# Nicolo2277/Vivim

Measured on AMD Instinct MI355X. Metric: frames/sec fwd+bwd, 256x256 clip=5 3-class, higher is better.
Workload: dtype bf16

## Files before the change

### vivim_amd/_lib.py

```python
import collections
import ctypes
import os
import re
import subprocess

import torch

_HERE = os.path.dirname(os.path.abspath(__file__))
CSRC = os.path.join(_HERE, "csrc")
SO_PATH = os.environ.get("VIVIM_LIB") or os.path.join(CSRC, "libvivim_hip.so")
HEADER = os.path.join(os.path.dirname(_HERE), "include", "vivim_hip.h")

i32, i64, vp = ctypes.c_int32, ctypes.c_int64, ctypes.c_void_p

STRUCT_NAMES = {
    "vivim_ssm_fwd_params": "SsmFwdParams", "vivim_ssm_bwd_params": "SsmBwdParams",
    "vivim_conv_fwd_params": "ConvFwdParams", "vivim_conv_bwd_params": "ConvBwdParams",
    "vivim_dwconv_params": "DwConvParams", "vivim_dwconv_wgrad_params": "DwConvWgradParams",
    "vivim_dir_params": "DirParams", "vivim_conv_update_params": "ConvUpdateParams",
    "vivim_state_update_params": "StateUpdateParams", "vivim_layernorm_params": "LayerNormParams",
    "vivim_wgrad_nt_params": "WgradNtParams", "vivim_add_layernorm_params": "AddLayerNormParams",
    "vivim_seg_loss_params": "SegLossParams", "vivim_seg_metrics_params": "SegMetricsParams",
    "vivim_upsample_params": "UpsampleParams",
    "vivim_decode_head_params": "DecodeHeadParams", "vivim_token_layernorm_params": "TokenLayerNormParams",
    "vivim_token_add_norm_params": "TokenAddNormParams", "vivim_opt_step_params": "OptStepParams",
    "vivim_opt_mw_params": "OptMwParams",
}
EXTENSIONS = {"vivim_hip_ext.h": ({"vivim_structure_loss_params": "StructureLossParams"}, {}),
              "vivim_hip_ext_head.h": ({"vivim_head_concat_params": "HeadConcatParams"}, {}),
              "vivim_hip_ext_binary_metrics.h": ({"vivim_binary_metrics_params": "BinaryMetricsParams"}, {})}

Entry = collections.namedtuple("Entry", "struct extra stream restype")

_FIELD_TYPES = {"int32_t": i32, "int64_t": i64, "float": ctypes.c_float, "double": ctypes.c_double,
                "void *": vp, "const void *": vp, "const void *const *": ctypes.POINTER(vp),
                "const int64_t *": ctypes.POINTER(i64)}
_ARG_TYPES = {"void *": vp, "size_t": ctypes.c_size_t, "int": ctypes.c_int}
_RESTYPES = {"int": ctypes.c_int, "size_t": ctypes.c_size_t, "const char *": ctypes.c_char_p}
_DIRECTIVES = r"\s*#\s*(include|define|ifndef\s+VIVIM_HIP(_[A-Z0-9]+)*_H|endif)\b"


def _refuse(header, what, text):
    raise ValueError(f"{header}: {what}: {' '.join(text.split())!r}")


def _ctype(text):
    return re.sub(r"\s*\*\s*", " *", " ".join(text.split()))


def _declarator(text, table, context, header):
    m = re.fullmatch(r"([\w\s*]*?)(\w+)\s*(?:\[\s*(\d+)\s*\])?", text.strip())
    if not m:
        _refuse(header, "cannot parse the declarator", context)
    if _ctype(m[1]) not in table:
        _refuse(header, f"unknown type {_ctype(m[1])!r}", context)
    ctype = table[_ctype(m[1])]
    return m[2], (ctype * int(m[3]) if m[3] else ctype)


def _has_sizeof_row(cls):
    return cls._fields_[0][0] != "struct_bytes"


def parse_header(text, names=STRUCT_NAMES, header="vivim_hip.h"):
    text = re.sub(r"/\*.*?\*/", " ", text, flags=re.S)
    consts = {k: int(v) for k, v in re.findall(r"^[ \t]*#[ \t]*define[ \t]+(VIVIM_\w+)[ \t]+(-?\d+)[ \t]*$", text, flags=re.M)}
    by_c_name = {}

    def struct(m):
        body, c_name = m[1], m[2]
        if "{" in body or "#" in body:
            _refuse(header, "nested braces or a preprocessor line in a struct", m[0])
        if c_name not in names:
            _refuse(header, "a struct without a Python name in STRUCT_NAMES", c_name)
        types = {**_FIELD_TYPES, **by_c_name}
        fields = []
        for stmt in filter(None, (s.strip() for s in body.split(";"))):
            base = re.match(r"(?:const\s+)?\w+", stmt) or _refuse(header, "cannot parse the field", stmt)
            first, *more = stmt.split(",")
            for decl in [first] + [f"{base[0]} {d}" for d in more]:
                fields.append(_declarator(decl, types, stmt, header))
        by_c_name[c_name] = type(names[c_name], (ctypes.Structure,), {"_fields_": fields, "__module__": __name__})
        return " "

    def enum(m):
        for item in filter(None, (s.strip() for s in m[1].split(","))):
            kv = re.fullmatch(r"(\w+)\s*=\s*(-?\d+)", item) or _refuse(header, "cannot parse the enumerator", item)
            consts[kv[1]] = int(kv[2])
        return " "

    text = re.sub(r"typedef\s+struct\s*\{(.*?)\}\s*(\w+)\s*;", struct, text, flags=re.S)
    text = re.sub(r"(?:typedef\s+)?enum\s*\{([^{}]*)\}\s*\w*\s*;", enum, text)
    missing = [c for c in names if c not in by_c_name]
    if missing:
        _refuse(header, "STRUCT_NAMES names structs the header does not have", ", ".join(missing))
    text = re.sub(r"^[ \t]*#[ \t]*ifdef[ \t]+__cplusplus\b.*?^[ \t]*#[ \t]*endif\b", " ", text, flags=re.S | re.M)
    for line in re.findall(r"^[ \t]*#.*$", text, flags=re.M):
        if not re.match(_DIRECTIVES, line):
            _refuse(header, "a preprocessor line it does not know", line)
    text = re.sub(r"^[ \t]*#.*$", " ", text, flags=re.M)

    entries = {}
    for decl in filter(None, (s.strip() for s in text.split(";"))):
        m = re.fullmatch(r"([\w\s*]+?)(\w+)\s*\(([\w\s*,]*)\)", decl) or _refuse(header, "cannot parse the declaration", decl)
        if _ctype(m[1]) not in _RESTYPES:
            _refuse(header, f"unknown return type {_ctype(m[1])!r}", decl)
        args = [] if m[3].strip() == "void" else [a.strip() for a in m[3].split(",")]
        stream = bool(args) and re.fullmatch(r"void\s*\*\s*stream", args[-1]) is not None
        args = args[:-1] if stream else args
        params, extra = None, []
        for k, arg in enumerate(args):
            p = re.fullmatch(r"const\s+(vivim_\w+)\s*\*\s*\w+", arg) if k == 0 else None
            if not p:
                extra.append(_declarator(arg, _ARG_TYPES, decl, header)[1])
            elif p[1] not in by_c_name:
                _refuse(header, f"unknown struct {p[1]}", decl)
            elif _has_sizeof_row(by_c_name[p[1]]):
                params = by_c_name[p[1]]
            else:
                extra.append(ctypes.POINTER(by_c_name[p[1]]))
        entries[m[2]] = Entry(params, tuple(extra), stream, _RESTYPES[_ctype(m[1])])
    return consts, {names[c]: by_c_name[c] for c in names}, entries


def _read_header(path=None):
    path = path or HEADER
    try:
        with open(path) as f:
            return f.read()
    except OSError as e:
        raise ImportError(f"{path} cannot be read ({e}): the binding is derived from it") from e


def load_extensions(extensions, include_dir, taken_entries, taken_classes):
    classes, entries = {}, {}
    for file, (names, own) in extensions.items():
        _, new, parsed = parse_header(_read_header(os.path.join(include_dir, file)), names, file)
        bad = [f"{n} does not open with struct_bytes" for n, c in new.items() if _has_sizeof_row(c)]
        bad += [f"another header already declares {n}" for n in parsed if n in taken_entries or n in entries]
        bad += [f"the name {n} is already taken" for n in new if n in taken_classes or n in classes]
        if bad:
            raise ImportError(f"{file}: {'; '.join(bad)}")
        own.update(parsed)
        entries.update(parsed)
        classes.update(new)
    return classes, entries


_consts, _classes, ENTRY_POINTS = parse_header(_read_header())
globals().update(_classes)
STRUCTS = tuple(c for c in _classes.values() if _has_sizeof_row(c))
EXPORTS = tuple(ENTRY_POINTS)
ABI_VERSION = _consts["VIVIM_ABI_VERSION"]
F32, F16, BF16 = _consts["VIVIM_F32"], _consts["VIVIM_F16"], _consts["VIVIM_BF16"]
OPT_CHUNK, OPT_MAX_TENSORS, OPT_STATE_WORDS = (_consts["VIVIM_OPT_" + n] for n in ("CHUNK", "MAX_TENSORS", "STATE_WORDS"))
_classes, _entries = load_extensions(EXTENSIONS, os.path.dirname(HEADER), ENTRY_POINTS, globals())
globals().update(_classes)
ALL_ENTRY_POINTS = {**ENTRY_POINTS, **_entries}

_lib = None


def build(force=False):
    if force:
        subprocess.check_call(["make", "-C", CSRC, "clean"])
    subprocess.check_call(["make", "-C", CSRC, "-j4"])
    return SO_PATH


def lib():
    global _lib
    if _lib is None:
        if not os.path.exists(SO_PATH):
            raise ImportError(
                f"{SO_PATH} is missing: run `python -c 'import __graft_entry__ as g; g.build()'` "
                "(or `make -C vivim_amd/csrc`). vivim_amd has no fallback path.")
        L = ctypes.CDLL(SO_PATH)
        for name, e in ALL_ENTRY_POINTS.items():
            fn = getattr(L, name)
            fn.argtypes = ([ctypes.POINTER(e.struct)] if e.struct else []) + list(e.extra) + ([vp] if e.stream else [])
            fn.restype = e.restype
        if L.vivim_abi_version() != ABI_VERSION:
            raise ImportError("libvivim_hip.so ABI version mismatch")
        for which, st in enumerate(STRUCTS):
            if L.vivim_sizeof(which) != ctypes.sizeof(st):
                raise ImportError(f"struct layout mismatch for {st.__name__}: "
                                  f"C {L.vivim_sizeof(which)} vs ctypes {ctypes.sizeof(st)}")
        _lib = L
    return _lib


_ISIZE = {F32: 4, F16: 2, BF16: 2}


def algorithmic_bytes(name, P):
    name = name.removesuffix("_det")
    f = P.f if isinstance(P, (SsmBwdParams, ConvBwdParams)) else P
    if name.startswith("vivim_opt"):
        if name.endswith("finalise"):
            return 8 * P.total_blocks + 4 * OPT_STATE_WORDS
        n = sum(P.numel[i] for i in range(P.count) if P.grads[i])
        if name.endswith("_mw"):
            return 2 * n + 8 * P.n_blocks if name.endswith("stats_mw") else 28 * n
        return 4 * n + 8 * P.n_blocks if name.endswith("stats") else 28 * n
    if name.startswith("vivim_add_layernorm"):
        n = P.batch * P.seqlen * P.channels
        if not P.weight:
            return n * ((2 if name.endswith("fwd") else 1) * _ISIZE[P.itype] + _ISIZE[P.btype])
        if name.endswith("fwd"):
            return n * (2 * _ISIZE[P.itype] + _ISIZE[P.btype] + _ISIZE[P.otype]) + 8 * P.batch * P.seqlen + 8 * P.channels
        res = (_ISIZE[P.itype] if P.dres else 0) + (_ISIZE[P.otype] if P.dy else 0) + (_ISIZE[P.btype] if P.dbranch else 0)
        return n * (2 * _ISIZE[P.itype] + res) + 8 * P.batch * P.seqlen + 12 * P.channels
    if name.startswith("vivim_token_add_norm"):
        n, b, r = P.rows * P.channels, _ISIZE[P.btype], _ISIZE[P.rtype]
        stats = 8 * P.rows if P.mean and P.weight else 0
        small = (4 * (P.rows // P.rows_per_sample) if P.scale else 0) + (4 * P.channels if P.weight else 0)
        if name.endswith("fwd"):
            small += 4 * P.channels if P.weight and P.bias else 0
            return n * (b + (r if P.res else 0) + (r if P.res_out else 0) + (b if P.weight else 0)) + stats + small
        norm = bool(P.weight and P.dy)
        small += (4 * P.channels if norm and P.dweight else 0) + (4 * P.channels if norm and P.dbias else 0)
        return (n * ((r + b if norm else 0) + (r if P.dres else 0) + (r if P.dres_in else 0) + (b if P.dbranch else 0))
                + (stats if norm else 0) + small)
    if name.startswith("vivim_token_layernorm"):
        n = P.rows * P.channels
        stats = 8 * P.rows if P.mean else 0
        if name.endswith("fwd"):
            return n * (_ISIZE[P.itype] + _ISIZE[P.otype]) + stats
        return n * (2 * _ISIZE[P.itype] + _ISIZE[P.otype]) + stats + 12 * P.channels
    if name.startswith("vivim_decode_head"):
        px = sum(P.map_h[s] * P.map_w[s] for s in range(P.n_maps))
        return (P.batch * (px * P.hidden + P.classes * P.out_h * P.out_w) * _ISIZE[P.itype]
                + 4 * (P.hidden + P.classes * P.hidden + P.classes))
    if name.startswith("vivim_head_concat"):
        px = P.out_h * P.out_w
        maps = sum(P.map_c[s] * (P.map_h[s] * P.map_w[s] + px) for s in range(P.n_maps)) * _ISIZE[P.itype]
        return P.batch * (maps + sum(P.map_c[s] * px for s in range(P.n_maps) if P.keep[s]))
    if name.startswith("vivim_upsample"):
        return P.batch * P.channels * (P.in_h * P.in_w + P.out_h * P.out_w) * _ISIZE[P.itype]
    if name.startswith("vivim_seg_metrics"):
        n = P.batch * P.pixels
        return n * (P.classes * _ISIZE[P.itype] + (8 if P.ttype == 0 else 1) + (1 if P.pred else 0)) + 12 * P.batch * P.classes
    if name.startswith("vivim_structure_loss"):
        n = P.batch * P.height * P.width
        return (n * ((2 if name.endswith("bwd") else 1) * P.classes * _ISIZE[P.itype] + (8 if P.ttype == 0 else 1))
                + 12 * P.batch * P.classes)
    if name.startswith("vivim_seg_loss"):
        n = P.batch * P.pixels
        return (n * ((2 if name.endswith("bwd") else 1) * P.classes * _ISIZE[P.itype] + (8 if P.ttype == 0 else 1))
                + 8 * P.batch * P.classes)
    if name.startswith("vivim_binary_metrics"):
        n = P.batch * P.height * P.width
        return (3 * n * (_ISIZE[P.ptype] + _ISIZE.get(P.gtype, 1)) + P.batch * (72 + (4096 if P.hist else 0))
                + (160 if P.state else 0))
    if name.startswith("vivim_selective_scan"):
        s = _ISIZE[f.itype]
        act = f.batch * f.dim * f.seqlen * s
        bc = (f.batch * f.n_groups * f.dstate * f.seqlen) if f.is_variable_B else f.dim * f.dstate
        has_z = bool(f.z)
        if name.endswith("fwd_lean"):
            return (4 if has_z else 3) * act + 2 * bc * (s if f.is_variable_B else 4) + 4 * (f.dim * f.dstate + 2 * f.dim)
        if name.endswith("fwd"):
            n_act = 3 + (2 if has_z else 0)
            return n_act * act + 2 * bc * (s if f.is_variable_B else 4) + 4 * (f.dim * f.dstate + 2 * f.dim)
        n_act = 5 + (3 if has_z else 0) + (1 if (has_z and f.out_z) else 0)
        return (n_act * act + 2 * bc * (s if f.is_variable_B else 4) + 2 * bc * 4
                + 4 * (2 * f.dim * f.dstate + 4 * f.dim))
    if name.endswith("_update"):
        return 0
    if name.startswith("vivim_dir"):
        return 4 * P.batch * P.channels * P.seqlen * _ISIZE[P.itype]
    if name.startswith("vivim_dwconv"):
# ... 136 lines not shown
```

### vivim_amd/dirmap.py

```python
import torch

from . import _lib
from ._lib import ITYPE


def _params(flat, stacked, nframes, csplit, scale, src, dst):
    B, C, L = flat.shape
    P = _lib.DirParams()
    P.batch, P.channels, P.seqlen, P.nframes, P.csplit, P.itype, P.scale = B, C, L, nframes, csplit, ITYPE[flat.dtype], scale
    P.flat_batch_stride, P.flat_c_stride = flat.stride(0), flat.stride(1)
    P.stk_batch_stride, P.stk_half_stride, P.stk_dir_stride, P.stk_c_stride = (stacked.stride(0), stacked.stride(1),
                                                                               stacked.stride(2), stacked.stride(3))
    P.src, P.dst = src.data_ptr(), dst.data_ptr()
    return P


def _scatter(flat, nframes, csplit, scale):
    if flat.stride(-1) != 1:
        flat = flat.contiguous()
    B, C, L = flat.shape
    stacked = _lib.empty((C // csplit, 3, csplit, B, L), flat.dtype, flat.device).permute(3, 0, 1, 2, 4)
    _lib.launch("vivim_dir_scatter", _params(flat, stacked, nframes, csplit, scale, flat, stacked), flat.device)
    return stacked


def _gather(stacked, nframes, scale, channel_major=False):
    if stacked.stride(-1) != 1:
        stacked = stacked.contiguous()
    B, H, _, csplit, L = stacked.shape
    if channel_major:
        flat = _lib.empty((H * csplit, B, L), stacked.dtype, stacked.device).permute(1, 0, 2)
    else:
        flat = _lib.empty((B, H * csplit, L), stacked.dtype, stacked.device)
    _lib.launch("vivim_dir_gather", _params(flat, stacked, nframes, csplit, scale, stacked, flat), stacked.device)
    return flat


class _StackFn(torch.autograd.Function):
    @staticmethod
    def forward(ctx, xz, nframes, halves):
        ctx.nframes = nframes
        return _scatter(xz, nframes, xz.shape[1] // halves, 1.0)

    @staticmethod
    def backward(ctx, g):
        return _gather(g, ctx.nframes, 1.0), None, None


class _CombineFn(torch.autograd.Function):
    @staticmethod
    def forward(ctx, o3, nframes):
        ctx.nframes = nframes
        B, _, D, L = o3.shape
        return _gather(o3.view(B, 1, 3, D, L), nframes, 1.0 / 3.0, channel_major=True)

    @staticmethod
    def backward(ctx, g):
        B, D, L = g.shape
        return _scatter(g, ctx.nframes, D, 1.0 / 3.0).view(B, 3, D, L), None


def stack_directions(xz, nframes, halves=2):
    return _StackFn.apply(xz, nframes, halves)


def combine_directions(o3, nframes):
    return _CombineFn.apply(o3, nframes)
```

### vivim_amd/dwconv.py

```python
import os

import torch

from . import _lib
from ._lib import ITYPE, ptr


def supported(x, weight):
    if os.environ.get("VIVIM_NO_DWCONV") or not (x.is_cuda and x.dim() == 3 and x.dtype in ITYPE and x.stride(2) == 1):
        return False
    cv = 16 // x.element_size()
    ks = tuple(weight.shape[2:])
    return (weight.shape[1] == 1 and ks in ((3, 3), (3, 3, 3)) and x.shape[2] % cv == 0
            and x.stride(1) % cv == 0 and x.stride(0) % cv == 0 and x.data_ptr() % 16 == 0)


def _taps(weight):
    C = weight.shape[0]
    return weight.detach().reshape(C, -1).t().contiguous().float()


def _aligned(t):
    cv = 16 // t.element_size()
    if t.stride(2) != 1 or t.data_ptr() % 16 or t.stride(1) % cv or t.stride(0) % cv:
# ... 8 lines not shown
    P = _lib.DwConvParams()
    P.batch, P.depth, P.height, P.width, P.channels = B, D, H, W, C
    P.kd, P.itype, P.flip = wt.shape[0] // 9, ITYPE[x.dtype], int(flip)
    P.x_batch_stride, P.x_token_stride = x.stride(0), x.stride(1)
    P.y_batch_stride, P.y_token_stride = y.stride(0), y.stride(1)
    P.x, P.wt, P.y = x.data_ptr(), wt.data_ptr(), y.data_ptr()
    P.bias = ptr(bias)
    P.act = act
    if aux is not None:
        P.aux, P.aux_batch_stride, P.aux_token_stride = aux.data_ptr(), aux.stride(0), aux.stride(1)
    _lib.launch("vivim_dwconv_fwd", P, x.device)
    return y


def _run_wgrad(x, dy, wt, dims, has_bias):
    B, L, C = x.shape
    D, H, W = dims
    acc = _lib.zeros(wt.shape[0] * C + C, x.device)
    P = _lib.DwConvWgradParams()
    P.batch, P.depth, P.height, P.width, P.channels = B, D, H, W, C
    P.kd, P.itype = wt.shape[0] // 9, ITYPE[x.dtype]
    P.x_batch_stride, P.x_token_stride = x.stride(0), x.stride(1)
    P.dy_batch_stride, P.dy_token_stride = dy.stride(0), dy.stride(1)
    P.x, P.dy, P.dwt = x.data_ptr(), dy.data_ptr(), acc.data_ptr()
    P.dbias = acc.data_ptr() + 4 * wt.shape[0] * C if has_bias else None
    if _lib.deterministic():
        nbytes, ws = _lib.workspace("vivim_dwconv_wgrad_det_workspace_bytes", P, x.device)
        _lib.launch("vivim_dwconv_wgrad_det", P, x.device, ptr(ws), nbytes)
    else:
        _lib.launch("vivim_dwconv_wgrad", P, x.device)
    return acc


class DepthwiseConvTokensFn(torch.autograd.Function):
    @staticmethod
    def forward(ctx, x, weight, bias, D, H, W):
        assert x.shape[1] == D * H * W, "token count must equal D*H*W"
        wt = _taps(weight)
        ctx.save_for_backward(x, wt)
        ctx.dims, ctx.wshape, ctx.wdtype = (D, H, W), weight.shape, weight.dtype
        ctx.has_bias = bias is not None
        ctx.bias_dtype = bias.dtype if bias is not None else None
        return _run_fwd(x, wt, bias.detach().float().contiguous() if bias is not None else None, (D, H, W), False)

    @staticmethod
    def backward(ctx, dy):
        x, wt = ctx.saved_tensors
        D, H, W = ctx.dims
        dy = _aligned(dy)
        dx = _run_fwd(dy, wt, None, (D, H, W), True) if ctx.needs_input_grad[0] else None
        C = x.shape[2]
        acc = _run_wgrad(x, dy, wt, (D, H, W), ctx.has_bias)
        dweight = acc[:wt.shape[0] * C].view(wt.shape[0], C).t().reshape(ctx.wshape).to(ctx.wdtype)
        dbias = acc[wt.shape[0] * C:].to(ctx.bias_dtype) if ctx.has_bias else None
        return dx, dweight, dbias, None, None, None


class DepthwiseConvGeluTokensFn(torch.autograd.Function):

    @staticmethod
    def forward(ctx, x, weight, bias, D, H, W):
        assert x.shape[1] == D * H * W, "token count must equal D*H*W"
        wt = _taps(weight)
        bf = bias.detach().float().contiguous() if bias is not None else None
        ctx.save_for_backward(x, wt, bf)
        ctx.dims, ctx.wshape, ctx.wdtype = (D, H, W), weight.shape, weight.dtype
        ctx.bias_dtype = bias.dtype if bias is not None else None
        return _run_fwd(x, wt, bf, (D, H, W), False, act=1)

    @staticmethod
    def backward(ctx, dy):
        x, wt, bf = ctx.saved_tensors
        dims = ctx.dims
        dpre = _run_fwd(x, wt, bf, dims, False, act=2, aux=_aligned(dy))
        dx = _run_fwd(dpre, wt, None, dims, True) if ctx.needs_input_grad[0] else None
        C = x.shape[2]
        acc = _run_wgrad(x, dpre, wt, dims, bf is not None)
        dweight = acc[:wt.shape[0] * C].view(wt.shape[0], C).t().reshape(ctx.wshape).to(ctx.wdtype)
        dbias = acc[wt.shape[0] * C:].to(ctx.bias_dtype) if bf is not None else None
        return dx, dweight, dbias, None, None, None


def depthwise_conv_tokens(x, weight, bias, D, H, W):
    return DepthwiseConvTokensFn.apply(x, weight, bias, D, H, W)


def depthwise_conv_gelu_tokens(x, weight, bias, D, H, W):
    return DepthwiseConvGeluTokensFn.apply(x, weight, bias, D, H, W)
```

### vivim_amd/layernorm.py

```python
import ctypes

import torch

from . import _lib
from ._lib import ITYPE, ptr


def supported(x, weight):
    if _lib.deterministic():
        return False
    if not (x.is_cuda and x.dim() == 3 and x.dtype in ITYPE and weight is not None and weight.dtype == torch.float32):
        return False
    B, L, C = x.shape
    e = 16 // x.element_size()
    return (x.stride(1) == 1 and C <= 512 and L % e == 0 and x.stride(0) % e == 0 and x.stride(2) % e == 0
            and x.data_ptr() % 16 == 0 and x.stride(2) >= L)


def worthwhile(x):
    return x.shape[0] * x.shape[1] >= 4096


def _params(x, out_dtype, eps):
    B, L, C = x.shape
    P = _lib.LayerNormParams()
    P.batch, P.seqlen, P.channels, P.itype, P.otype, P.eps = B, L, C, ITYPE[x.dtype], ITYPE[out_dtype], eps
    P.x_batch_stride, P.x_c_stride = x.stride(0), x.stride(2)
    P.x = x.data_ptr()
    return P


def _norm_forward(P, x, weight, bias, out_dtype):
    B, L, C = x.shape
    y = _lib.empty((B, L, C), out_dtype, x.device)
    stats = _lib.empty((2, B, L), torch.float32, x.device)
    P.y_batch_stride, P.y_token_stride = L * C, C
    P.weight, P.bias = weight.data_ptr(), ptr(bias)
    P.y, P.mean = y.data_ptr(), stats.data_ptr()
    P.rstd = P.mean + 4 * B * L
    return y, stats


def _norm_backward(P, query, dy, weight, stats, out_dtype, has_bias):
    B, L, C = P.batch, P.seqlen, P.channels
    P.weight, P.mean = weight.data_ptr(), stats.data_ptr()
    P.rstd = P.mean + 4 * B * L
    if dy is None:
        return None, None
    if dy.dtype != out_dtype:
        dy = dy.to(out_dtype)
    if dy.stride(2) != 1 or dy.stride(1) < C:
        dy = dy.contiguous()
    P.dy, P.y_batch_stride, P.y_token_stride = dy.data_ptr(), dy.stride(0), dy.stride(1)
    dwb = _lib.zeros(2 * C, stats.device)
    P.dweight = dwb.data_ptr()
    P.dbias = P.dweight + 4 * C if has_bias else None
    ws = _lib.workspace(query, P, stats.device)[1]
    P.workspace = ptr(ws)
    return dwb, (dy, ws)


class _LayerNormCM(torch.autograd.Function):
    @staticmethod
    def forward(ctx, x, weight, bias, eps, out_dtype):
        P = _params(x, out_dtype, eps)
        y, stats = _norm_forward(P, x, weight, bias, out_dtype)
        _lib.launch("vivim_layernorm_cm_fwd", P, x.device)
        ctx.save_for_backward(x, weight, stats)
        ctx.eps, ctx.has_bias, ctx.out_dtype = eps, bias is not None, out_dtype
        return y

    @staticmethod
    def backward(ctx, dy):
        x, weight, stats = ctx.saved_tensors
        B, L, C = x.shape
        dx = _lib.empty((B, C, L), x.dtype, x.device).transpose(1, 2)
        P = _params(x, ctx.out_dtype, ctx.eps)
        P.dx, P.dx_batch_stride, P.dx_c_stride = dx.data_ptr(), C * L, L
        dwb, _alive = _norm_backward(P, "vivim_layernorm_bwd_workspace_bytes", dy, weight, stats, ctx.out_dtype, ctx.has_bias)
        _lib.launch("vivim_layernorm_cm_bwd", P, x.device)
        return dx, dwb[:C], (dwb[C:] if ctx.has_bias else None), None, None


def layer_norm_cm(x, weight, bias, eps=1e-5, out_dtype=None):
    if out_dtype is None:
        out_dtype = torch.float32 if torch.is_autocast_enabled() else x.dtype
    return _LayerNormCM.apply(x, weight, bias, eps, out_dtype)


def _cm_ok(t, e):
    return (t.stride(1) == 1 and t.shape[1] % e == 0 and t.stride(0) % e == 0 and t.stride(2) % e == 0
            and t.data_ptr() % 16 == 0 and t.stride(2) >= t.shape[1])


def add_norm_supported(x, branch, weight=None):
    if _lib.deterministic():
        return False
    if not (x.is_cuda and x.dim() == 3 and x.dtype in ITYPE and branch.device == x.device and branch.shape == x.shape):
        return False
    if weight is not None and weight.dtype != torch.float32:
        return False
    if not (branch.dtype == x.dtype or (x.dtype == torch.float32 and branch.dtype in (torch.float16, torch.bfloat16))):
        return False
    C = x.shape[2]
    return C <= 512 and _cm_ok(x, 16 // x.element_size()) and branch.stride(2) == 1 and branch.stride(1) >= C


def _add_params(x, branch, scale):
    B, L, C = x.shape
    P = _lib.AddLayerNormParams()
    P.batch, P.seqlen, P.channels, P.itype, P.btype, P.otype = B, L, C, ITYPE[x.dtype], ITYPE[branch.dtype], ITYPE[x.dtype]
    P.scale = ptr(scale)
    return P


def _check_scale(scale, x):
    if scale is not None and not (scale.dtype == torch.float32 and scale.shape == (x.shape[0],) and scale.is_contiguous()
                                  and scale.device == x.device):
        raise ValueError("scale must be a contiguous (batch,) float32 tensor on x's device")


def _as_cm(g, like):
    if g.dtype != like.dtype:
        g = g.to(like.dtype)
    if not _cm_ok(g, 16 // g.element_size()):
        g = g.transpose(1, 2).contiguous().transpose(1, 2)
    return g


def _add_forward(x, branch, scale, P):
    B, L, C = x.shape
    x_new = _lib.empty((B, C, L), x.dtype, x.device).transpose(1, 2)
    P.x_batch_stride, P.x_c_stride = x.stride(0), x.stride(2)
    P.x_new_batch_stride, P.x_new_c_stride = C * L, L
    P.branch_batch_stride, P.branch_token_stride = branch.stride(0), branch.stride(1)
    P.x, P.branch, P.x_new = x.data_ptr(), branch.data_ptr(), x_new.data_ptr()
    return x_new


class _AddLayerNormCM(torch.autograd.Function):
    @staticmethod
    def forward(ctx, x, branch, weight, bias, scale, eps, out_dtype):
        P = _add_params(x, branch, scale)
        P.otype, P.eps = ITYPE[out_dtype], eps
        x_new = _add_forward(x, branch, scale, P)
        y, stats = _norm_forward(P, x, weight, bias, out_dtype)
        _lib.launch("vivim_add_layernorm_cm_fwd", P, x.device)
        ctx.save_for_backward(x_new, weight, stats, scale)
        ctx.eps, ctx.has_bias, ctx.out_dtype, ctx.branch_dtype = eps, bias is not None, out_dtype, branch.dtype
        ctx.set_materialize_grads(False)
        return x_new, y

    @staticmethod
    def backward(ctx, dres, dy):
        if dres is None and dy is None:
            return (None,) * 7
        x_new, weight, stats, scale = ctx.saved_tensors
        B, L, C = x_new.shape
        P = _lib.AddLayerNormParams()
        P.batch, P.seqlen, P.channels, P.eps = B, L, C, ctx.eps
        P.itype, P.btype, P.otype = ITYPE[x_new.dtype], ITYPE[ctx.branch_dtype], ITYPE[ctx.out_dtype]
        P.scale = ptr(scale)
        P.x_new_batch_stride, P.x_new_c_stride = x_new.stride(0), x_new.stride(2)
        P.x_new = x_new.data_ptr()
        dwb, _alive = _norm_backward(P, "vivim_add_layernorm_bwd_workspace_bytes", dy, weight, stats, ctx.out_dtype, ctx.has_bias)
        if dres is not None:
            dres = _as_cm(dres, x_new)
            P.dres, P.dres_batch_stride, P.dres_c_stride = dres.data_ptr(), dres.stride(0), dres.stride(2)
        dx = _lib.empty((B, C, L), x_new.dtype, x_new.device).transpose(1, 2)
# ... 358 lines not shown
```

### vivim_amd/mamba_simple.py

```python
import math

import torch
import torch.nn as nn
import torch.nn.functional as F

import os

from .dirmap import combine_directions, stack_directions
from .causal_conv1d_interface import causal_conv1d_fn, causal_conv1d_update
from .selective_scan_interface import mamba_inner_fn_no_out_proj, mamba_inner_grouped_fn_no_out_proj, selective_scan_fn
from .selective_state_update import selective_state_update

_DIRECTIONS = ("", "_b", "_s")
_FUSED = ("conv1d{}.weight", "conv1d{}.bias", "x_proj{}.weight", "dt_proj{}.weight", "dt_proj{}.bias", "A{}_log", "D{}")


class _FusedViews(torch.autograd.Function):

    @staticmethod
    def forward(ctx, nb, *args):
        ctx.nb = nb
        return tuple(b.view_as(b) for b in args[:nb])

    @staticmethod
    def backward(ctx, *gs):
        out = [None] * (1 + ctx.nb)
        for g in gs:
            out += [None, None, None] if g is None else [g[0], g[1], g[2]]
        return tuple(out)


class Mamba(nn.Module):
    def __init__(self, d_model, d_state=16, d_conv=4, expand=2, dt_rank="auto", dt_min=0.001, dt_max=0.1,
                 dt_init="random", dt_scale=1.0, dt_init_floor=1e-4, conv_bias=True, bias=False,
                 use_fast_path=True, layer_idx=None, device=None, dtype=None, bimamba_type="none",
                 nframes=5):
        kw = {"device": device, "dtype": dtype}
        super().__init__()
        assert bimamba_type == "v3", "this fork only builds the tri-directional v3 block (mamba_simple.py:125)"
        self.d_model, self.d_state, self.d_conv, self.expand = d_model, d_state, d_conv, expand
        self.d_inner = int(expand * d_model)
        self.dt_rank = math.ceil(d_model / 16) if dt_rank == "auto" else dt_rank
        self.use_fast_path = use_fast_path
        self.layer_idx = layer_idx
        self.bimamba_type = bimamba_type
        self.nframes = nframes
        self.activation = "silu"

        self.in_proj = nn.Linear(d_model, 2 * self.d_inner, bias=bias, **kw)
        for sfx in _DIRECTIONS:
            self.add_module("conv1d" + sfx, nn.Conv1d(self.d_inner, self.d_inner, kernel_size=d_conv,
                                                      groups=self.d_inner, padding=d_conv - 1,
                                                      bias=conv_bias, **kw))
            self.add_module("x_proj" + sfx, nn.Linear(self.d_inner, self.dt_rank + 2 * d_state, bias=False, **kw))
            dt_proj = nn.Linear(self.dt_rank, self.d_inner, bias=True, **kw)
            self.add_module("dt_proj" + sfx, dt_proj)
            if sfx == "":
                std = self.dt_rank ** -0.5 * dt_scale
                if dt_init == "constant":
                    nn.init.constant_(dt_proj.weight, std)
                elif dt_init == "random":
                    nn.init.uniform_(dt_proj.weight, -std, std)
                else:
                    raise NotImplementedError
                dt = torch.exp(torch.rand(self.d_inner, **kw) * (math.log(dt_max) - math.log(dt_min))
                               + math.log(dt_min)).clamp(min=dt_init_floor)
                with torch.no_grad():
                    dt_proj.bias.copy_(dt + torch.log(-torch.expm1(-dt)))
                dt_proj.bias._no_reinit = True
            A_log = torch.log(torch.arange(1, d_state + 1, dtype=torch.float32, device=device)
                              ).repeat(self.d_inner, 1).contiguous()
            a_name = f"A{sfx}_log"
            self.register_parameter(a_name, nn.Parameter(A_log))
            getattr(self, a_name)._no_weight_decay = True
            d_name = "D" + sfx
            self.register_parameter(d_name, nn.Parameter(torch.ones(self.d_inner, device=device)))
            getattr(self, d_name)._no_weight_decay = True
        self.out_proj = nn.Linear(self.d_inner, d_model, bias=bias, **kw)

    def _fuse(self):
        def param(path):
            obj = self
            for name in path.split("."):
                obj = getattr(obj, name)
            return obj
        bufs, groups = [], []
        for kind in _FUSED:
            ps = [param(kind.format(sfx)) for sfx in _DIRECTIONS]
            if any(p is None for p in ps):
                bufs.append(None)
                groups.append(None)
                continue
            buf = torch.stack([p.data for p in ps])
            for g, p in enumerate(ps):
                p.data = buf[g]
            bufs.append(buf)
            groups.append(ps)
        self._fused = bufs
        self._fused_live = [b for b in bufs if b is not None]
        self._fused_args = self._fused_live + [p for ps in groups if ps is not None for p in ps]
        self._fused_where = []
        for kind, buf in zip(_FUSED, bufs):
            if buf is None:
                continue
            for g, sfx in enumerate(_DIRECTIONS):
                *mods, attr = kind.format(sfx).split(".")
                owner = self
                for name in mods:
                    owner = getattr(owner, name)
                self._fused_where.append((owner._parameters, attr, buf[g].data_ptr(), buf.dtype, buf.device))

    def _fused_params(self):
        where = getattr(self, "_fused_where", None)
        ok = where is not None
        if ok:
            args = self._fused_args
            k = len(self._fused_live)
            for i, (params, attr, ptr, dtype, device) in enumerate(where):
                prm = params.get(attr)
                if prm is not args[k + i] or prm.data_ptr() != ptr or prm.dtype != dtype or prm.device != device:
                    ok = False
                    break
        if not ok:
            self._fuse()
        bufs = self._fused
        views = iter(_FusedViews.apply(len(self._fused_live), *self._fused_args))
        return [None if b is None else next(views) for b in bufs]

    def _inner(self, xz, sfx):
        conv, x_proj, dt_proj = (getattr(self, n + sfx) for n in ("conv1d", "x_proj", "dt_proj"))
        A = -torch.exp(getattr(self, f"A{sfx}_log").float())
        return mamba_inner_fn_no_out_proj(
            xz, conv.weight, conv.bias, x_proj.weight, dt_proj.weight, A, None, None,
            getattr(self, "D" + sfx).float(), delta_bias=dt_proj.bias.float(), delta_softplus=True)

    def forward(self, hidden_states, inference_params=None, nframes=None):
        batch, seqlen, _ = hidden_states.shape
        if inference_params is not None:
            conv_state, ssm_state = self._get_states_from_cache(inference_params, batch)
            if inference_params.seqlen_offset > 0:
                return self.step(hidden_states, conv_state, ssm_state)[0]
            return self._prefill(hidden_states, conv_state, ssm_state)
        nf = self.nframes if nframes is None else nframes
        if seqlen % nf != 0:
            raise ValueError(f"seqlen {seqlen} is not a multiple of nframes {nf}")
        xz = (self.in_proj.weight @ hidden_states.reshape(batch * seqlen, -1).t()
              ).view(2 * self.d_inner, batch, seqlen).transpose(0, 1)
        if self.in_proj.bias is not None:
            xz = xz + self.in_proj.bias.to(xz.dtype)[:, None]
        hw = seqlen // nf
        if os.environ.get("VIVIM_SEPARATE_DIRECTIONS", "0") == "1" or seqlen % 8 != 0:
            return self._forward_separate(xz, batch, seqlen, nf, hw)
        D = self.d_inner
        xz3 = stack_directions(xz, nf)
        conv_w, conv_b, x_proj_w, dt_proj_w, dt_bias, A_log, Dp = self._fused_params()
        A = -torch.exp(A_log.float()).view(3 * D, self.d_state)
        o3 = mamba_inner_grouped_fn_no_out_proj(
            xz3, conv_w.view(3 * D, self.d_conv), conv_b.view(3 * D) if conv_b is not None else None, x_proj_w, dt_proj_w,
            A, Dp.float().view(3 * D), dt_bias.float().view(3 * D), True).view(batch, 3, D, seqlen)
        y = combine_directions(o3, nf).transpose(1, 2)
        return F.linear(y, self.out_proj.weight, self.out_proj.bias)

    def _prefill(self, hidden_states, conv_state, ssm_state):
        batch, seqlen, _ = hidden_states.shape
        xz = (self.in_proj.weight @ hidden_states.reshape(batch * seqlen, -1).t()
              ).view(2 * self.d_inner, batch, seqlen).transpose(0, 1)
        if self.in_proj.bias is not None:
            xz = xz + self.in_proj.bias.to(xz.dtype)[:, None]
        x, z = xz.chunk(2, dim=1)
        with torch.no_grad():
            k = min(seqlen, self.d_conv)
            conv_state.zero_()
            conv_state[:, :, self.d_conv - k:].copy_(x[:, :, seqlen - k:])
        x = causal_conv1d_fn(x, self.conv1d.weight.squeeze(1), self.conv1d.bias, self.activation)
        x_dbl = self.x_proj(x.transpose(1, 2).reshape(batch * seqlen, self.d_inner))
        dt, B, C = torch.split(x_dbl, [self.dt_rank, self.d_state, self.d_state], dim=-1)
        dt = (self.dt_proj.weight @ dt.t()).view(self.d_inner, batch, seqlen).transpose(0, 1)
        B = B.reshape(batch, seqlen, self.d_state).transpose(1, 2).contiguous()
        C = C.reshape(batch, seqlen, self.d_state).transpose(1, 2).contiguous()
        y, last_state = selective_scan_fn(x, dt, -torch.exp(self.A_log.float()), B, C, self.D.float(), z=z,
                                          delta_bias=self.dt_proj.bias.float(), delta_softplus=True, return_last_state=True)
        with torch.no_grad():
            ssm_state.copy_(last_state)
        return self.out_proj(y.transpose(1, 2))

    def _get_states_from_cache(self, inference_params, batch_size, initialize_states=False):
        assert self.layer_idx is not None
        if self.layer_idx not in inference_params.key_value_memory_dict:
            inference_params.key_value_memory_dict[self.layer_idx] = self.allocate_inference_cache(batch_size, 0)
        conv_state, ssm_state = inference_params.key_value_memory_dict[self.layer_idx]
        if initialize_states:
            conv_state.zero_()
            ssm_state.zero_()
        return conv_state, ssm_state

    def _forward_separate(self, xz, batch, seqlen, nf, hw):
        out = self._inner(xz, "")
        out_b = self._inner(xz.flip([-1]), "_b").flip([-1])
        xz_s = xz.reshape(batch, 2 * self.d_inner, nf, hw).transpose(2, 3).reshape(batch, 2 * self.d_inner, seqlen)
        out_s = self._inner(xz_s, "_s")
        out_s = out_s.reshape(batch, self.d_inner, hw, nf).transpose(2, 3).reshape(batch, self.d_inner, seqlen)
        y = (out + out_b + out_s).transpose(1, 2) / 3
        return F.linear(y, self.out_proj.weight, self.out_proj.bias)

    def step(self, hidden_states, conv_state, ssm_state):
        assert hidden_states.shape[1] == 1, "Only support decoding with 1 token at a time for now"
        xz = self.in_proj(hidden_states.squeeze(1))
        x, z = xz.chunk(2, dim=-1)
        x = causal_conv1d_update(x.contiguous(), conv_state, self.conv1d.weight.squeeze(1), self.conv1d.bias, self.activation)
# ... 15 lines not shown
```

Before: 235.9.

## Move autograd nodes for dwconv, direction maps, LayerNorm and fused views into C++

```diff
diff --git a/vivim_amd/_lib.py b/vivim_amd/_lib.py
--- a/vivim_amd/_lib.py
+++ b/vivim_amd/_lib.py
@@ -3,6 +3,7 @@
 import os
 import re
 import subprocess
+import sys
 
 import torch
 
@@ -158,13 +159,16 @@
 globals().update(_classes)
 ALL_ENTRY_POINTS = {**ENTRY_POINTS, **_entries}
 
+NODES_PATH = os.path.join(CSRC, "_vivim_nodes.so")
+
 _lib = None
+_nodes = None
 
 
 def build(force=False):
     if force:
         subprocess.check_call(["make", "-C", CSRC, "clean"])
-    subprocess.check_call(["make", "-C", CSRC, "-j4"])
+    subprocess.check_call(["make", "-C", CSRC, "-j4", "PYTHON=" + sys.executable])
     return SO_PATH
 
 
@@ -188,6 +192,39 @@
                                   f"C {L.vivim_sizeof(which)} vs ctypes {ctypes.sizeof(st)}")
         _lib = L
     return _lib
+
+
+def nodes():
+    global _nodes
+    if _nodes is None:
+        lib()
+        if not os.path.exists(NODES_PATH):
+            raise ImportError(
+                f"{NODES_PATH} is missing: run `python -c 'import __graft_entry__ as g; g.build()'` "
+                "(or `make -C vivim_amd/csrc`). vivim_amd has no fallback path.")
+        import importlib.util
+        spec = importlib.util.spec_from_file_location("_vivim_nodes", NODES_PATH)
+        mod = importlib.util.module_from_spec(spec)
+        spec.loader.exec_module(mod)
+        if mod.abi_version != ABI_VERSION or mod.torch_version != torch.__version__.split("+")[0]:
+            raise ImportError(f"{NODES_PATH} was built for ABI version {mod.abi_version} and torch {mod.torch_version}, not "
+                              f"{ABI_VERSION} and {torch.__version__}: rebuild it (`make -C vivim_amd/csrc`)")
+        _nodes = mod
+    return _nodes
+
+
+_cpp_nodes = os.environ.get("VIVIM_NO_CPP_NODES", "0") in ("0", "") and not os.environ.get("VIVIM_LIB")
+
+
+def cpp_nodes(on):
+    global _cpp_nodes
+    prev, _cpp_nodes = _cpp_nodes, bool(on)
+    return prev
+
+
+def use_cpp_nodes(x):
+    return (_cpp_nodes and not GUARD and (_profile is None or not _profile[1]) and x.is_cuda
+            and x.device.index == torch.cuda.current_device())
 
 
 _ISIZE = {F32: 4, F16: 2, BF16: 2}
diff --git a/vivim_amd/csrc/nodes_flags.py b/vivim_amd/csrc/nodes_flags.py
--- /dev/null
+++ b/vivim_amd/csrc/nodes_flags.py
@@ -0,0 +1,14 @@
+import sys
+import sysconfig
+
+import torch
+from torch.utils import cpp_extension
+
+if sys.argv[1:] == ["compile"]:
+    paths = [sysconfig.get_paths()["include"]] + cpp_extension.include_paths()
+    print(" ".join(f"-isystem {p}" for p in paths), f"-D_GLIBCXX_USE_CXX11_ABI={int(torch._C._GLIBCXX_USE_CXX11_ABI)}")
+elif sys.argv[1:] == ["link"]:
+    libs = ("torch", "torch_cpu", "torch_python", "c10", "c10_hip", "torch_hip")
+    print(" ".join(f"-L{p} -Wl,-rpath,{p}" for p in cpp_extension.library_paths()), " ".join("-l" + n for n in libs))
+else:
+    sys.exit("usage: nodes_flags.py compile|link")
diff --git a/vivim_amd/csrc/torch_nodes.cpp b/vivim_amd/csrc/torch_nodes.cpp
--- /dev/null
+++ b/vivim_amd/csrc/torch_nodes.cpp
@@ -0,0 +1,424 @@
+#include <torch/extension.h>
+
+#include <c10/hip/HIPStream.h>
+#include <torch/csrc/DynamicTypes.h>
+#include <torch/csrc/autograd/python_cpp_function.h>
+#include <torch/csrc/autograd/python_variable.h>
+
+#include <cstring>
+#include <stdexcept>
+#include <string>
+#include <vector>
+
+#include "vivim_hip.h"
+#include "vivim_hip_ext.h"
+#include "vivim_hip_ext_binary_metrics.h"
+#include "vivim_hip_ext_head.h"
+
+namespace {
+
+using at::Tensor;
+using torch::autograd::AutogradContext;
+using torch::autograd::variable_list;
+using OptTensor = c10::optional<Tensor>;
+
+int itype_of(at::ScalarType t) {
+    switch (t) {
+    case at::kFloat: return VIVIM_F32;
+    case at::kHalf: return VIVIM_F16;
+    case at::kBFloat16: return VIVIM_BF16;
+    default: {
+        py::gil_scoped_acquire gil;
+        PyErr_SetObject(PyExc_KeyError, reinterpret_cast<PyObject *>(torch::getTHPDtype(t)));
+        throw py::error_already_set();
+    }
+    }
+}
+
+at::ScalarType dtype_of(int64_t itype) {
+    switch (itype) {
+    case VIVIM_F32: return at::kFloat;
+    case VIVIM_F16: return at::kHalf;
+    case VIVIM_BF16: return at::kBFloat16;
+    default: throw std::invalid_argument("itype must be VIVIM_F32, VIVIM_F16 or VIVIM_BF16");
+    }
+}
+
+const void *ptr(const Tensor &t) { return t.defined() ? t.data_ptr() : nullptr; }
+
+const Tensor &value_or_undefined(const OptTensor &t) {
+    static const Tensor undefined;
+    return t.has_value() ? *t : undefined;
+}
+
+void check_rc(int rc) {
+    if (rc != 0)
+        throw std::runtime_error(vivim_last_error());
+}
+
+void *stream_of(const Tensor &t) { return c10::hip::getCurrentHIPStream(t.get_device()).stream(); }
+
+template <class P> void zero(P &p) { std::memset(&p, 0, sizeof(P)); }
+
+void fill_dwconv(vivim_dwconv_params &P, const Tensor &x, const Tensor &wt, const Tensor &bias, const Tensor &y, int64_t D,
+                 int64_t H, int64_t W, bool flip, int act, const Tensor &aux) {
+    zero(P);
+    P.batch = (int32_t)x.size(0), P.depth = (int32_t)D, P.height = (int32_t)H, P.width = (int32_t)W, P.channels = (int32_t)x.size(2);
+    P.kd = (int32_t)(wt.size(0) / 9), P.itype = itype_of(x.scalar_type()), P.flip = flip;
+    P.x_batch_stride = x.stride(0), P.x_token_stride = x.stride(1);
+    P.y_batch_stride = y.stride(0), P.y_token_stride = y.stride(1);
+    P.x = x.data_ptr(), P.wt = wt.data_ptr(), P.y = y.data_ptr();
+    P.bias = ptr(bias);
+    P.act = act;
+    if (aux.defined())
+        P.aux = aux.data_ptr(), P.aux_batch_stride = aux.stride(0), P.aux_token_stride = aux.stride(1);
+}
+
+void fill_dwconv_wgrad(vivim_dwconv_wgrad_params &P, const Tensor &x, const Tensor &dy, const Tensor &acc, int64_t taps, int64_t D,
+                       int64_t H, int64_t W, bool has_bias) {
+    zero(P);
+    const int64_t C = x.size(2);
+    P.batch = (int32_t)x.size(0), P.depth = (int32_t)D, P.height = (int32_t)H, P.width = (int32_t)W, P.channels = (int32_t)C;
+    P.kd = (int32_t)(taps / 9), P.itype = itype_of(x.scalar_type());
+    P.x_batch_stride = x.stride(0), P.x_token_stride = x.stride(1);
+    P.dy_batch_stride = dy.stride(0), P.dy_token_stride = dy.stride(1);
+    P.x = x.data_ptr(), P.dy = dy.data_ptr(), P.dwt = acc.data_ptr();
+    P.dbias = has_bias ? static_cast<char *>(acc.data_ptr()) + 4 * taps * C : nullptr;
+}
+
+Tensor taps_of(const Tensor &weight) {
+    return weight.detach().reshape({weight.size(0), -1}).t().contiguous().to(at::kFloat);
+}
+
+Tensor aligned(const Tensor &t) {
+    const int64_t cv = 16 / t.element_size();
+    if (t.stride(2) != 1 || reinterpret_cast<uintptr_t>(t.data_ptr()) % 16 || t.stride(1) % cv || t.stride(0) % cv)
+        return t.contiguous();
+    return t;
+}
+
+Tensor dwconv_run_fwd(const Tensor &x, const Tensor &wt, const Tensor &bias, int64_t D, int64_t H, int64_t W, bool flip, int act,
+                      const Tensor &aux) {
+    Tensor y = at::empty({x.size(0), x.size(1), x.size(2)}, x.options());
+    vivim_dwconv_params P;
+    fill_dwconv(P, x, wt, bias, y, D, H, W, flip, act, aux);
+    check_rc(vivim_dwconv_fwd(&P, stream_of(x)));
+    return y;
+}
+
+Tensor dwconv_run_wgrad(const Tensor &x, const Tensor &dy, const Tensor &wt, int64_t D, int64_t H, int64_t W, bool has_bias) {
+    const int64_t C = x.size(2), taps = wt.size(0);
+    Tensor acc = at::zeros({taps * C + C}, x.options().dtype(at::kFloat));
+    vivim_dwconv_wgrad_params P;
+    fill_dwconv_wgrad(P, x, dy, acc, taps, D, H, W, has_bias);
+    if (at::globalContext().deterministicAlgorithms()) {
+        const size_t nbytes = vivim_dwconv_wgrad_det_workspace_bytes(&P);
+        Tensor ws;
+        if (nbytes)
+            ws = at::empty({(int64_t)nbytes}, x.options().dtype(at::kByte));
+        check_rc(vivim_dwconv_wgrad_det(&P, ws.defined() ? ws.data_ptr() : nullptr, nbytes, stream_of(x)));
+    } else {
+        check_rc(vivim_dwconv_wgrad(&P, stream_of(x)));
+    }
+    return acc;
+}
+
+struct DwConvFn : torch::autograd::Function<DwConvFn> {
+    static Tensor forward(AutogradContext *ctx, const Tensor &x, const Tensor &weight, const OptTensor &bias, int64_t D, int64_t H,
+                          int64_t W, bool gelu) {
+        if (x.size(1) != D * H * W) {
+            PyErr_SetString(PyExc_AssertionError, "token count must equal D*H*W");
+            throw py::error_already_set();
+        }
+        Tensor wt = taps_of(weight), bf;
+        if (bias.has_value())
+            bf = bias->detach().to(at::kFloat).contiguous();
+        if (gelu)
+            ctx->save_for_backward({x, wt, bf});
+        else
+            ctx->save_for_backward({x, wt});
+        ctx->saved_data["dims"] = std::vector<int64_t>{D, H, W, gelu, bias.has_value(), (int64_t)weight.scalar_type(),
+                                                       (int64_t)(bias.has_value() ? bias->scalar_type() : at::kFloat)};
+        ctx->saved_data["wshape"] = weight.sizes().vec();
+        return dwconv_run_fwd(x, wt, bf, D, H, W, false, gelu ? 1 : 0, Tensor());
+    }
+
+    static variable_list backward(AutogradContext *ctx, variable_list grads) {
+        const variable_list saved = ctx->get_saved_variables();
+        const Tensor &x = saved[0], &wt = saved[1];
+        const std::vector<int64_t> dims = ctx->saved_data["dims"].toIntVector();
+        const int64_t D = dims[0], H = dims[1], W = dims[2];
+        const bool gelu = dims[3], has_bias = dims[4];
+        Tensor dy = aligned(grads[0]);
+        if (gelu)
+            dy = dwconv_run_fwd(x, wt, saved[2], D, H, W, false, 2, dy);
+        Tensor dx;
+        if (ctx->needs_input_grad(0))
+            dx = dwconv_run_fwd(dy, wt, Tensor(), D, H, W, true, 0, Tensor());
+        const int64_t C = x.size(2), taps = wt.size(0);
+        Tensor acc = dwconv_run_wgrad(x, dy, wt, D, H, W, has_bias);
+        Tensor dweight = acc.slice(0, 0, taps * C).view({taps, C}).t().reshape(ctx->saved_data["wshape"].toIntVector())
+                             .to((at::ScalarType)dims[5]);
+        Tensor dbias;
+        if (has_bias)
+            dbias = acc.slice(0, taps * C).to((at::ScalarType)dims[6]);
+        return {dx, dweight, dbias, Tensor(), Tensor(), Tensor(), Tensor()};
+    }
+};
+
+void fill_dir(vivim_dir_params &P, const Tensor &flat, const Tensor &stacked, int64_t nframes, int64_t csplit, double scale,
+              bool scatter) {
+    zero(P);
+    P.batch = (int32_t)flat.size(0), P.channels = (int32_t)flat.size(1), P.seqlen = (int32_t)flat.size(2);
+    P.nframes = (int32_t)nframes, P.csplit = (int32_t)csplit, P.itype = itype_of(flat.scalar_type()), P.scale = (float)scale;
+    P.flat_batch_stride = flat.stride(0), P.flat_c_stride = flat.stride(1);
+    P.stk_batch_stride = stacked.stride(0), P.stk_half_stride = stacked.stride(1);
+    P.stk_dir_stride = stacked.stride(2), P.stk_c_stride = stacked.stride(3);
+    P.src = scatter ? flat.data_ptr() : stacked.data_ptr();
+    P.dst = scatter ? stacked.data_ptr() : flat.data_ptr();
+}
+
+Tensor dir_scatter(Tensor flat, int64_t nframes, int64_t csplit, double scale) {
+    if (flat.stride(-1) != 1)
+        flat = flat.contiguous();
+    const int64_t B = flat.size(0), C = flat.size(1), L = flat.size(2);
+    Tensor stacked = at::empty({C / csplit, 3, csplit, B, L}, flat.options()).permute({3, 0, 1, 2, 4});
+    vivim_dir_params P;
+    fill_dir(P, flat, stacked, nframes, csplit, scale, true);
+    check_rc(vivim_dir_scatter(&P, stream_of(flat)));
+    return stacked;
+}
+
+Tensor dir_gather(Tensor stacked, int64_t nframes, double scale, bool channel_major) {
+    if (stacked.stride(-1) != 1)
+        stacked = stacked.contiguous();
+    const int64_t B = stacked.size(0), Hh = stacked.size(1), csplit = stacked.size(3), L = stacked.size(4);
+    Tensor flat = channel_major ? at::empty({Hh * csplit, B, L}, stacked.options()).permute({1, 0, 2})
+                                : at::empty({B, Hh * csplit, L}, stacked.options());
+    vivim_dir_params P;
+    fill_dir(P, flat, stacked, nframes, csplit, scale, false);
+    check_rc(vivim_dir_gather(&P, stream_of(stacked)));
+    return flat;
+}
+
+struct StackFn : torch::autograd::Function<StackFn> {
+    static Tensor forward(AutogradContext *ctx, const Tensor &xz, int64_t nframes, int64_t halves) {
+        ctx->saved_data["nframes"] = nframes;
+        return dir_scatter(xz, nframes, xz.size(1) / halves, 1.0);
+    }
+    static variable_list backward(AutogradContext *ctx, variable_list grads) {
+        return {dir_gather(grads[0], ctx->saved_data["nframes"].toInt(), 1.0, false), Tensor(), Tensor()};
+    }
+};
+
+struct CombineFn : torch::autograd::Function<CombineFn> {
+    static Tensor forward(AutogradContext *ctx, const Tensor &o3, int64_t nframes) {
+        ctx->saved_data["nframes"] = nframes;
+        const int64_t B = o3.size(0), D = o3.size(2), L = o3.size(3);
+        return dir_gather(o3.view({B, 1, 3, D, L}), nframes, 1.0 / 3.0, true);
+    }
+    static variable_list backward(AutogradContext *ctx, variable_list grads) {
+        const Tensor &g = grads[0];
+        const int64_t B = g.size(0), D = g.size(1), L = g.size(2);
+        return {dir_scatter(g, ctx->saved_data["nframes"].toInt(), D, 1.0 / 3.0).view({B, 3, D, L}), Tensor()};
+    }
+};
+
+struct FusedViewsFn : torch::autograd::Function<FusedViewsFn> {
+    static variable_list forward(AutogradContext *ctx, int64_t nb, at::TensorList args) {
+        ctx->saved_data["nb"] = nb;
+        variable_list out;
+        out.reserve(nb);
+        for (int64_t i = 0; i < nb; ++i)
+            out.push_back(args[i].view_as(args[i]));
+        return out;
+    }
+    static variable_list backward(AutogradContext *ctx, variable_list grads) {
+        const int64_t nb = ctx->saved_data["nb"].toInt();
+        variable_list out(1 + nb);
+        out.reserve(1 + 4 * nb);
+        for (const Tensor &g : grads)
+            for (int64_t k = 0; k < 3; ++k)
+                out.push_back(g.defined() ? g.select(0, k) : Tensor());
+        return out;
+    }
+};
+
+void fill_layernorm(vivim_layernorm_params &P, const Tensor &x, at::ScalarType out_dtype, double eps) {
+    zero(P);
+    P.batch = (int32_t)x.size(0), P.seqlen = (int32_t)x.size(1), P.channels = (int32_t)x.size(2);
+    P.itype = itype_of(x.scalar_type()), P.otype = itype_of(out_dtype), P.eps = (float)eps;
+    P.x_batch_stride = x.stride(0), P.x_c_stride = x.stride(2);
+    P.x = x.data_ptr();
+}
+
+void fill_layernorm_fwd(vivim_layernorm_params &P, const Tensor &x, const Tensor &weight, const Tensor &bias, const Tensor &y,
+                        const Tensor &stats, at::ScalarType out_dtype, double eps) {
+    fill_layernorm(P, x, out_dtype, eps);
+    const int64_t B = x.size(0), L = x.size(1), C = x.size(2);
+    P.y_batch_stride = L * C, P.y_token_stride = C;
+    P.weight = weight.data_ptr(), P.bias = ptr(bias);
+    P.y = y.data_ptr(), P.mean = stats.data_ptr();
+    P.rstd = static_cast<char *>(stats.data_ptr()) + 4 * B * L;
+}
+
+void fill_layernorm_bwd(vivim_layernorm_params &P, const Tensor &x, const Tensor &weight, const Tensor &stats, const Tensor &dy,
+                        const Tensor &dx, const Tensor &dwb, const Tensor &ws, at::ScalarType out_dtype, double eps, bool has_bias) {
+    fill_layernorm(P, x, out_dtype, eps);
+    const int64_t B = x.size(0), L = x.size(1), C = x.size(2);
+    P.dx = dx.data_ptr(), P.dx_batch_stride = C * L, P.dx_c_stride = L;
+    P.weight = weight.data_ptr(), P.mean = stats.data_ptr();
+    P.rstd = static_cast<char *>(stats.data_ptr()) + 4 * B * L;
+    P.dy = dy.data_ptr(), P.y_batch_stride = dy.stride(0), P.y_token_stride = dy.stride(1);
+    P.dweight = dwb.data_ptr();
+    P.dbias = has_bias ? static_cast<char *>(dwb.data_ptr()) + 4 * C : nullptr;
+    P.workspace = ws.defined() ? ws.data_ptr() : nullptr;
+}
+
+struct LayerNormCMFn : torch::autograd::Function<LayerNormCMFn> {
+    static Tensor forward(AutogradContext *ctx, const Tensor &x, const Tensor &weight, const OptTensor &bias, double eps,
+                          int64_t otype) {
+        const at::ScalarType out_dtype = dtype_of(otype);
+        const int64_t B = x.size(0), L = x.size(1), C = x.size(2);
+        Tensor y = at::empty({B, L, C}, x.options().dtype(out_dtype));
+        Tensor stats = at::empty({2, B, L}, x.options().dtype(at::kFloat));
+        vivim_layernorm_params P;
+        fill_layernorm_fwd(P, x, weight, value_or_undefined(bias), y, stats, out_dtype, eps);
+        check_rc(vivim_layernorm_cm_fwd(&P, stream_of(x)));
+        ctx->save_for_backward({x, weight, stats});
+        ctx->saved_data["eps"] = eps;
+        ctx->saved_data["flags"] = std::vector<int64_t>{otype, bias.has_value()};
+        return y;
+    }
+
+    static variable_list backward(AutogradContext *ctx, variable_list grads) {
+        const variable_list saved = ctx->get_saved_variables();
+        const Tensor &x = saved[0], &weight = saved[1], &stats = saved[2];
+        const std::vector<int64_t> flags = ctx->saved_data["flags"].toIntVector();
+        const at::ScalarType out_dtype = dtype_of(flags[0]);
+        const bool has_bias = flags[1];
+        const int64_t B = x.size(0), L = x.size(1), C = x.size(2);
+        Tensor dx = at::empty({B, C, L}, x.options()).transpose(1, 2);
+        Tensor dy = grads[0];
+        if (dy.scalar_type() != out_dtype)
+            dy = dy.to(out_dtype);
+        if (dy.stride(2) != 1 || dy.stride(1) < C)
+            dy = dy.contiguous();
+        Tensor dwb = at::zeros({2 * C}, stats.options());
+        vivim_layernorm_params P;
+        fill_layernorm_bwd(P, x, weight, stats, dy, dx, dwb, Tensor(), out_dtype, ctx->saved_data["eps"].toDouble(), has_bias);
+        const size_t nbytes = vivim_layernorm_bwd_workspace_bytes(&P);
+        Tensor ws;
+        if (nbytes) {
+            ws = at::empty({(int64_t)nbytes}, stats.options().dtype(at::kByte));
+            P.workspace = ws.data_ptr();
+        }
+        check_rc(vivim_layernorm_cm_bwd(&P, stream_of(x)));
+        return {dx, dwb.slice(0, 0, C), has_bias ? dwb.slice(0, C) : Tensor(), Tensor(), Tensor()};
+    }
+};
+
+template <class Fn> PyObject *saved_tensors_of(PyObject *self, void *) {
+    HANDLE_TH_ERRORS
+    auto *node = static_cast<torch::autograd::CppNode<Fn> *>(reinterpret_cast<torch::autograd::THPCppFunction *>(self)->cdata.get());
+    const variable_list saved = node->ctx_.get_saved_variables();
+    THPObjectPtr tuple(PyTuple_New((Py_ssize_t)saved.size()));
+    if (!tuple)
+        return nullptr;
+    for (size_t i = 0; i < saved.size(); ++i) {
+        PyObject *item = saved[i].defined() ? THPVariable_Wrap(saved[i]) : Py_NewRef(Py_None);
+        if (!item)
+            return nullptr;
+        PyTuple_SET_ITEM(tuple.get(), (Py_ssize_t)i, item);
+    }
+    return tuple.release();
+    END_HANDLE_TH_ERRORS
+}
+
+template <class Fn> void register_node_class(const char *name) {
+    using namespace torch::autograd;
+    static PyTypeObject type;
+    static PyGetSetDef properties[] = {THP_FUNCTION_DEFAULT_PROPERTIES,
+                                       {(char *)"saved_tensors", saved_tensors_of<Fn>, nullptr, nullptr, nullptr},
+                                       {nullptr, nullptr, nullptr, nullptr, nullptr}};
+    torch::autograd::_initFunctionPyTypeObject(type, name, properties, nullptr);
+    torch::autograd::registerCppFunction(typeid(torch::autograd::CppNode<Fn>), &type);
+}
+
+template <class P> py::bytes bytes_of(const P &p) { return py::bytes(reinterpret_cast<const char *>(&p), sizeof(P)); }
+
+template <class P> const P *params_of(const std::string &bytes) {
+    if (bytes.size() != sizeof(P))
+        throw std::invalid_argument("the bytes are not one params struct of this entry point");
+    return reinterpret_cast<const P *>(bytes.data());
+}
+
+void debug_call(const std::string &name, const std::string &bytes) {
+    if (name == "vivim_dwconv_fwd")
+        check_rc(vivim_dwconv_fwd(params_of<vivim_dwconv_params>(bytes), nullptr));
+    else if (name == "vivim_dwconv_wgrad")
+        check_rc(vivim_dwconv_wgrad(params_of<vivim_dwconv_wgrad_params>(bytes), nullptr));
+    else if (name == "vivim_dir_scatter")
+        check_rc(vivim_dir_scatter(params_of<vivim_dir_params>(bytes), nullptr));
+    else if (name == "vivim_dir_gather")
+        check_rc(vivim_dir_gather(params_of<vivim_dir_params>(bytes), nullptr));
+    else if (name == "vivim_layernorm_cm_fwd")
+        check_rc(vivim_layernorm_cm_fwd(params_of<vivim_layernorm_params>(bytes), nullptr));
+    else if (name == "vivim_layernorm_cm_bwd")
+        check_rc(vivim_layernorm_cm_bwd(params_of<vivim_layernorm_params>(bytes), nullptr));
+    else
+        throw std::invalid_argument("debug_call: " + name + " is not an entry point of these nodes");
+}
+
+}
+
+PYBIND11_MODULE(TORCH_EXTENSION_NAME, m) {
+    m.doc() = "C++ autograd nodes of vivim_amd's depthwise-conv, direction-map and channel-major LayerNorm ops";
+    m.attr("torch_version") = TORCH_VERSION;
+    m.attr("abi_version") = VIVIM_ABI_VERSION;
+    register_node_class<DwConvFn>("DepthwiseConvTokensBackward");
+    register_node_class<StackFn>("StackDirectionsBackward");
+    register_node_class<CombineFn>("CombineDirectionsBackward");
+    register_node_class<FusedViewsFn>("FusedViewsBackward");
+    register_node_class<LayerNormCMFn>("LayerNormCMBackward");
+    m.def("dwconv", [](const Tensor &x, const Tensor &weight, const OptTensor &bias, int64_t D, int64_t H, int64_t W, bool gelu) {
+        return DwConvFn::apply(x, weight, bias, D, H, W, gelu);
+    });
+    m.def("stack_directions", [](const Tensor &xz, int64_t nframes, int64_t halves) { return StackFn::apply(xz, nframes, halves); });
+    m.def("combine_directions", [](const Tensor &o3, int64_t nframes) { return CombineFn::apply(o3, nframes); });
+    m.def("fused_views", [](int64_t nb, const std::vector<Tensor> &args) { return FusedViewsFn::apply(nb, at::TensorList(args)); });
+    m.def("layer_norm_cm", [](const Tensor &x, const Tensor &weight, const OptTensor &bias, double eps, int64_t otype) {
+        return LayerNormCMFn::apply(x, weight, bias, eps, otype);
+    });
+
+    m.def("fill_dwconv", [](const Tensor &x, const Tensor &wt, const OptTensor &bias, const Tensor &y, int64_t D, int64_t H, int64_t W,
+                            bool flip, int act, const OptTensor &aux) {
+        vivim_dwconv_params P;
+        fill_dwconv(P, x, wt, value_or_undefined(bias), y, D, H, W, flip, act, value_or_undefined(aux));
+        return bytes_of(P);
+    });
+    m.def("fill_dwconv_wgrad", [](const Tensor &x, const Tensor &dy, const Tensor &acc, int64_t taps, int64_t D, int64_t H, int64_t W,
+                                  bool has_bias) {
+        vivim_dwconv_wgrad_params P;
+        fill_dwconv_wgrad(P, x, dy, acc, taps, D, H, W, has_bias);
+        return bytes_of(P);
+    });
+    m.def("fill_dir", [](const Tensor &flat, const Tensor &stacked, int64_t nframes, int64_t csplit, double scale, bool scatter) {
+        vivim_dir_params P;
+        fill_dir(P, flat, stacked, nframes, csplit, scale, scatter);
+        return bytes_of(P);
+    });
+    m.def("fill_layernorm_fwd", [](const Tensor &x, const Tensor &weight, const OptTensor &bias, const Tensor &y, const Tensor &stats,
+                                   double eps, int64_t otype) {
+        vivim_layernorm_params P;
+        fill_layernorm_fwd(P, x, weight, value_or_undefined(bias), y, stats, dtype_of(otype), eps);
+        return bytes_of(P);
+    });
+    m.def("fill_layernorm_bwd", [](const Tensor &x, const Tensor &weight, const Tensor &stats, const Tensor &dy, const Tensor &dx,
+                                   const Tensor &dwb, const OptTensor &ws, double eps, int64_t otype, bool has_bias) {
+        vivim_layernorm_params P;
+        fill_layernorm_bwd(P, x, weight, stats, dy, dx, dwb, value_or_undefined(ws), dtype_of(otype), eps, has_bias);
+        return bytes_of(P);
+    });
+    m.def("debug_call", &debug_call);
+}
diff --git a/vivim_amd/dirmap.py b/vivim_amd/dirmap.py
--- a/vivim_amd/dirmap.py
+++ b/vivim_amd/dirmap.py
@@ -61,8 +61,12 @@
 
 
 def stack_directions(xz, nframes, halves=2):
+    if _lib.use_cpp_nodes(xz):
+        return _lib.nodes().stack_directions(xz, nframes, halves)
     return _StackFn.apply(xz, nframes, halves)
 
 
 def combine_directions(o3, nframes):
+    if _lib.use_cpp_nodes(o3):
+        return _lib.nodes().combine_directions(o3, nframes)
     return _CombineFn.apply(o3, nframes)
diff --git a/vivim_amd/dwconv.py b/vivim_amd/dwconv.py
--- a/vivim_amd/dwconv.py
+++ b/vivim_amd/dwconv.py
@@ -114,8 +114,12 @@
 
 
 def depthwise_conv_tokens(x, weight, bias, D, H, W):
+    if _lib.use_cpp_nodes(x):
+        return _lib.nodes().dwconv(x, weight, bias, D, H, W, False)
     return DepthwiseConvTokensFn.apply(x, weight, bias, D, H, W)
 
 
 def depthwise_conv_gelu_tokens(x, weight, bias, D, H, W):
+    if _lib.use_cpp_nodes(x):
+        return _lib.nodes().dwconv(x, weight, bias, D, H, W, True)
     return DepthwiseConvGeluTokensFn.apply(x, weight, bias, D, H, W)
diff --git a/vivim_amd/layernorm.py b/vivim_amd/layernorm.py
--- a/vivim_amd/layernorm.py
+++ b/vivim_amd/layernorm.py
@@ -85,6 +85,8 @@
 def layer_norm_cm(x, weight, bias, eps=1e-5, out_dtype=None):
     if out_dtype is None:
         out_dtype = torch.float32 if torch.is_autocast_enabled() else x.dtype
+    if _lib.use_cpp_nodes(x):
+        return _lib.nodes().layer_norm_cm(x, weight, bias, eps, ITYPE[out_dtype])
     return _LayerNormCM.apply(x, weight, bias, eps, out_dtype)
 
 
diff --git a/vivim_amd/mamba_simple.py b/vivim_amd/mamba_simple.py
--- a/vivim_amd/mamba_simple.py
+++ b/vivim_amd/mamba_simple.py
@@ -6,6 +6,7 @@
 
 import os
 
+from . import _lib
 from .dirmap import combine_directions, stack_directions
 from .causal_conv1d_interface import causal_conv1d_fn, causal_conv1d_update
 from .selective_scan_interface import mamba_inner_fn_no_out_proj, mamba_inner_grouped_fn_no_out_proj, selective_scan_fn
@@ -124,7 +125,10 @@
         if not ok:
             self._fuse()
         bufs = self._fused
-        views = iter(_FusedViews.apply(len(self._fused_live), *self._fused_args))
+        if _lib.use_cpp_nodes(self._fused_live[0]):
+            views = iter(_lib.nodes().fused_views(len(self._fused_live), self._fused_args))
+        else:
+            views = iter(_FusedViews.apply(len(self._fused_live), *self._fused_args))
         return [None if b is None else next(views) for b in bufs]
 
     def _inner(self, xz, sfx):
```

Measured after the change: 210.1. -10.9%, worse.
